# esologic/GANce

Hardware: AMD Instinct MI355X
Metric: synthesized frames/sec at 1024x1024 config-f (higher is better)
Workload: dtype f32 (bf16x3 split operands, 6 terms, fp32 accumulate)

## Files before the change

gance_amd/csrc/upfir_split.hip:

```cpp

#include <hip/hip_runtime.h>

#include <algorithm>
#include <cstdlib>
#include <cstring>
#include <type_traits>

#include "kernels.h"

#ifndef GANCE_UPFIRS_ABLATE
#define GANCE_UPFIRS_ABLATE 0
#endif

namespace gance {

namespace {

typedef float f32x4 __attribute__((ext_vector_type(4)));
typedef float f32x2 __attribute__((ext_vector_type(2)));
typedef unsigned u32x4 __attribute__((ext_vector_type(4)));
typedef __bf16 bf16x8 __attribute__((ext_vector_type(8)));
typedef __bf16 bf16x2 __attribute__((ext_vector_type(2)));
typedef __attribute__((address_space(3))) void* lds_ptr_t;

constexpr int kBM = 16;
constexpr int kKC = 32;
constexpr int kSW = 64;
constexpr int kTH = 8;
constexpr int kRows = kTH + 1;
constexpr int kPlanes = 12;
constexpr int kPlaneStride = 80;
constexpr int kSlotUnits = kPlanes * kPlaneStride;
constexpr int kRing = 3;
constexpr int kHaloCols = 4;
constexpr int kHaloUnits = kRows * kHaloCols * kPlanes;
constexpr int kHaloTasks = kRows * kHaloCols * 4;
#ifndef GANCE_UPFIRS_WEAVE
#define GANCE_UPFIRS_WEAVE 2
#endif
#ifndef GANCE_UPFIRS_MIN_SEG_ROWS
#define GANCE_UPFIRS_MIN_SEG_ROWS 16
#endif
#ifndef GANCE_UPFIRS_DEPTH
#define GANCE_UPFIRS_DEPTH 6
#endif
constexpr int kDepth = GANCE_UPFIRS_DEPTH;
constexpr int kCarryRows = 3;
constexpr int kPassCh = 4;
constexpr int kPassRows = 8;
constexpr int kTW = 2 * kSW + 4;
constexpr int kCG = kSW / 2;
constexpr int kRG = 64 / kCG;
constexpr int kFR = kPassRows / kRG;
constexpr int kWin = kFR + 3;
constexpr int kCarryFloats = kBM * kCarryRows * kTW;
constexpr int kStageFloats = kPassCh * kPassRows * kTW;
constexpr int kNzPieces = 2 * kPassRows * 2 * kSW / 256;
constexpr float kSqrt2f = 1.4142135623730951f;
static_assert((2 * kRows) % kDepth == 0 && kDepth + 2 < kRows && kRows % kRing == 0, "ring slots and staging registers rotate with the unrolled rows of a chunk pair");

constexpr size_t kRingBytes = (size_t)kRing * kSlotUnits * 16;
constexpr size_t kHaloBytes = (size_t)2 * kHaloUnits * 16;
constexpr int kWUnits = 27 * 64;
constexpr size_t kWBytes = (size_t)kWUnits * 16;
constexpr size_t lds_bytes(int cin) {
    return kRingBytes + kHaloBytes + kWBytes + sizeof(float) * ((size_t)kStageFloats + kNzPieces * 256 + kCarryFloats + cin + 3 * kBM);
}

__host__ __device__ constexpr int tap_cls(int t) { return t < 4 ? 0 : (t < 6 ? 1 : (t < 8 ? 2 : 3)); }
__host__ __device__ constexpr int tap_dy(int t) { return (t == 2 || t == 3 || t == 5) ? 1 : 0; }
__host__ __device__ constexpr int tap_dx(int t) { return (t == 1 || t == 3 || t == 7) ? 1 : 0; }

__device__ __forceinline__ void lds_barrier() {
    asm volatile("s_waitcnt lgkmcnt(0)" ::: "memory");
    __builtin_amdgcn_s_barrier();
    asm volatile("" ::: "memory");
}

__device__ __forceinline__ int fresh_lane() {
    int l;
    asm volatile("v_mbcnt_lo_u32_b32 %0, -1, 0\n\tv_mbcnt_hi_u32_b32 %0, -1, %0" : "=v"(l));
    return l;
}

__device__ __forceinline__ int ring_column(int P) {
    return ((P >> 2) & 3) | ((((P >> 4) ^ P) & 1) << 2) | (((P >> 1) & 1) << 3) | ((P & 1) << 4) | (P & 32);
}
constexpr int kEdgeColumn = 64;

__device__ __forceinline__ void split_pair(float a, float b, unsigned& p0, unsigned& p1, unsigned& p2) {
    auto pack = [](float lo, float hi) { return __builtin_bit_cast(unsigned, __builtin_convertvector(f32x2{lo, hi}, bf16x2)); };
    p0 = pack(a, b);
    const float ra = a - __builtin_bit_cast(float, p0 << 16), rb = b - __builtin_bit_cast(float, p0 & 0xffff0000u);
    p1 = pack(ra, rb);
    const float sa = ra - __builtin_bit_cast(float, p1 << 16), sb = rb - __builtin_bit_cast(float, p1 & 0xffff0000u);
    p2 = pack(sa, sb);
}

__device__ __forceinline__ void split_unit(const unsigned (&raw)[8], u32x4 (&part)[3]) {
    unsigned w[3][4];
    if (GANCE_UPFIRS_ABLATE & 1) {
#pragma unroll
        for (int q = 0; q < 3; ++q) part[q] = u32x4{raw[q], raw[q + 1], raw[q + 2], raw[q + 3]};
        return;
    }
#pragma unroll
    for (int e = 0; e < 4; ++e) split_pair(__builtin_bit_cast(float, raw[2 * e]), __builtin_bit_cast(float, raw[2 * e + 1]), w[0][e], w[1][e], w[2][e]);
#pragma unroll
    for (int q = 0; q < 3; ++q) part[q] = u32x4{w[q][0], w[q][1], w[q][2], w[q][3]};
}

}

template <bool kPre, bool kNoise>
__device__ __forceinline__ void upfirs_body(const UpFirArgs& p) {
    extern __shared__ __attribute__((aligned(16))) unsigned char smem_raw[];
    u32x4* const ring = reinterpret_cast<u32x4*>(smem_raw);
    u32x4* const halo = ring + kRing * kSlotUnits;
    u32x4* const w_lds = halo + 2 * kHaloUnits;
    float* const stage = reinterpret_cast<float*>(w_lds + kWUnits);
    float* const nz_lds = stage + kStageFloats;
    float* const carry = nz_lds + kNzPieces * 256;
    float* const s_lds = carry + kCarryFloats;
    float* const d_lds = s_lds + (kPre ? 0 : p.Cin);
    float* const b_lds = d_lds + kBM;
    float* const sn_lds = b_lds + kBM;

    const int tid = threadIdx.x;
    const int wave = __builtin_amdgcn_readfirstlane(tid >> 6);
    const int lane = tid & 63;
    const int n16 = lane & 15, kg = lane >> 4;

    int id;
    {
        const int v = blockIdx.x, nwg = p.total_blocks;
        const int q = nwg >> 3, r = nwg & 7, xcd = v & 7;
        id = (xcd < r ? xcd * (q + 1) : r * (q + 1) + (xcd - r) * q) + (v >> 3);
    }
    const int m_tile = id % p.m_tiles;
    id /= p.m_tiles;
    const int strip = id % p.strips;
    id /= p.strips;
    const int seg = id % p.segs;
    const int b = id / p.segs;
    const int m0 = m_tile * kBM;
    const int X0 = strip * kSW;
    const int H = p.H, W = p.W;
    const int Hp = H + 2, Wp = W + 8;
    const int HpWp4 = Hp * Wp * 4;
    const int chunks = p.Cin / kKC;
    const int steps = H / kTH;
    const int s_begin = seg * (p.rows_per_seg / kTH), s_end = s_begin + p.rows_per_seg / kTH;
    const int s_first = seg > 0 ? s_begin - 1 : s_begin;

    const __amdgpu_buffer_rsrc_t x_rsrc =
        __builtin_amdgcn_make_buffer_rsrc((void*)(p.x + (size_t)b * p.x_b_stride), 0, p.Cin * Hp * Wp * 4, 0x00020000);
    const __amdgpu_buffer_rsrc_t w_rsrc = __builtin_amdgcn_make_buffer_rsrc(
        (void*)(reinterpret_cast<const unsigned char*>(p.w) + (size_t)m_tile * chunks * 27 * 1024), 0, chunks * 27 * 1024, 0x00020000);

    const int st_pair = lane >> 4, st_g = lane & 15;
    u32x4* const ring_w = ring + wave * kPlaneStride + ring_column(4 * st_g + st_pair);
    const int m_pos = 16 * wave + n16;
    const u32x4* const ring_r0 = ring + kg * kPlaneStride + ring_column(m_pos);
    const u32x4* const ring_r1 = ring + kg * kPlaneStride + (m_pos > 0 ? ring_column(m_pos - 1) : kEdgeColumn);
    const bool edge_copy = wave == 3 && lane < kPlanes;
    const int e_unit = lane % kPlanes;
    u32x4* const ring_e = ring + (e_unit >> 2) * 4 * kPlaneStride + (e_unit & 3) * kPlaneStride + (edge_copy ? kEdgeColumn : 66 + wave);
    const u32x4* const halo_e = halo + e_unit;
    const u32x4* const halo_r = halo + ((n16 & 7) * kHaloCols + 2 * (n16 >> 3)) * kPlanes + kg;
    const u32x4* const halo_f = halo + ((kRows - 1) * kHaloCols + 2 * (n16 >> 3)) * kPlanes + kg;
    const int st_voff = (2 * st_pair * Hp * Wp + X0 + 4 + 4 * st_g) * 4;
    unsigned st[kDepth][8];
    auto stage_load = [&](unsigned(&dst)[8], int chunk, int brow, bool in_loop = false) {
        if ((GANCE_UPFIRS_ABLATE & 4) && in_loop) return;
        const int soff = ((chunk * kKC + wave * 8) * Hp + brow) * Wp * 4;
#pragma unroll
        for (int e = 0; e < 2; ++e) {
            const u32x4 q4 = __builtin_amdgcn_raw_buffer_load_b128(x_rsrc, st_voff, soff + e * HpWp4, 0);
#pragma unroll
            for (int c = 0; c < 4; ++c) dst[2 * c + e] = q4[c];
        }
    };
    auto scale_pair = [&](unsigned(&raw)[8], int chunk) {
        if constexpr (!kPre) {
            const f32x2 s2 = *reinterpret_cast<const f32x2*>(s_lds + chunk * kKC + 8 * wave + 2 * st_pair);
#pragma unroll
            for (int c = 0; c < 4; ++c) {
                raw[2 * c] = __builtin_bit_cast(unsigned, __builtin_bit_cast(float, raw[2 * c]) * s2[0]);
                raw[2 * c + 1] = __builtin_bit_cast(unsigned, __builtin_bit_cast(float, raw[2 * c + 1]) * s2[1]);
            }
        }
    };
    auto transpose_rows = [](u32x4& u) {
        auto a02 = __builtin_amdgcn_permlane32_swap(u[0], u[2], false, false);
        auto a13 = __builtin_amdgcn_permlane32_swap(u[1], u[3], false, false);
        auto b01 = __builtin_amdgcn_permlane16_swap(a02[0], a13[0], false, false);
        auto b23 = __builtin_amdgcn_permlane16_swap(a02[1], a13[1], false, false);
        u = u32x4{b01[0], b01[1], b23[0], b23[1]};
    };
    auto scale8 = [&](unsigned(&raw)[8], int chunk, int group) {
        if constexpr (!kPre) {
            const f32x4 s0 = *reinterpret_cast<const f32x4*>(s_lds + chunk * kKC + group * 8);
            const f32x4 s1 = *reinterpret_cast<const f32x4*>(s_lds + chunk * kKC + group * 8 + 4);
#pragma unroll
            for (int e = 0; e < 4; ++e) {
                raw[e] = __builtin_bit_cast(unsigned, __builtin_bit_cast(float, raw[e]) * s0[e]);
                raw[4 + e] = __builtin_bit_cast(unsigned, __builtin_bit_cast(float, raw[4 + e]) * s1[e]);
            }
        }
    };
    auto stage_store = [&](unsigned(&raw)[8], int slot, int chunk) {
        scale_pair(raw, chunk);
        u32x4 part[3];
        split_unit(raw, part);
#pragma unroll
        for (int q = 0; q < 3; ++q) transpose_rows(part[q]);
#pragma unroll
        for (int q = 0; q < 3; ++q)
            if (!(GANCE_UPFIRS_ABLATE & 16)) ring_w[slot * kSlotUnits + q * 4 * kPlaneStride] = part[q];
    };
    auto edge_store = [&](int slot, int hbuf, int hrow) { if (!(GANCE_UPFIRS_ABLATE & 64)) ring_e[slot * kSlotUnits] = halo_e[hbuf * kHaloUnits + (hrow * kHaloCols + 1) * kPlanes]; };
    const int h_task = tid < kHaloTasks ? tid : tid - kHaloTasks;
    const int h_col = h_task & 3, h_kg = (h_task >> 2) & 3, h_row = h_task >> 4;
    const int h_voff = ((h_kg * 8 * Hp + h_row) * Wp + X0 + 2 + (h_col & 1) + (h_col >> 1) * 65) * 4;
    u32x4* const halo_w = halo + (h_row * kHaloCols + h_col) * kPlanes + h_kg;
    unsigned hraw[8];
    auto halo_load = [&](int step, int chunk) {
        const int soff = (chunk * kKC * Hp + kTH * step) * Wp * 4;
#pragma unroll
        for (int e = 0; e < 8; ++e) hraw[e] = __builtin_amdgcn_raw_buffer_load_b32(x_rsrc, h_voff, soff + e * HpWp4, 0);
    };
    auto halo_store = [&](int chunk, int buf) {
        scale8(hraw, chunk, h_kg);
        u32x4 part[3];
        split_unit(hraw, part);
#pragma unroll
        for (int q = 0; q < 3; ++q) halo_w[buf * kHaloUnits + q * 4] = part[q];
    };

    u32x4 A[9][3];
    const int a_voff = lane * 16;
    auto weights_dma = [&](int chunk) {
#pragma unroll
        for (int k = 0; k < 7; ++k)
            if (k < 6 || wave < 3)
                __builtin_amdgcn_raw_ptr_buffer_load_lds(w_rsrc, (lds_ptr_t)(w_lds + (wave + 4 * k) * 64), 16, lane * 16, (chunk * 27 + wave + 4 * k) * 1024, 0, 0);
    };
    const u32x4* const w_r = w_lds + lane;
    auto read_a3 = [&](int t, u32x4(&dst)[3]) {
#pragma unroll
        for (int q = 0; q < 3; ++q) dst[q] = w_r[(t * 3 + q) * 64];
    };
    auto load_a3 = [&](int chunk, int t, u32x4(&dst)[3]) {
#pragma unroll
        for (int q = 0; q < 3; ++q) dst[q] = __builtin_amdgcn_raw_buffer_load_b128(w_rsrc, a_voff, (chunk * 27 + t * 3 + q) * 1024, 0);
    };

    u32x4 Bf[2][2][3];
    auto load_b = [&](int slot, u32x4(&dst)[2][3]) {
#pragma unroll
        for (int q = 0; q < 3; ++q) {
            dst[0][q] = ring_r0[slot * kSlotUnits + q * 4 * kPlaneStride];
            dst[1][q] = ring_r1[slot * kSlotUnits + q * 4 * kPlaneStride];
        }
    };

    stage_load(st[0], 0, kTH * s_first + 0);
    stage_load(st[1], 0, kTH * s_first + 1);
    load_a3(0, 0, A[0]);
    halo_load(s_first, 0);
    if constexpr (!kPre)
        for (int i = tid; i < p.Cin; i += 256) s_lds[i] = p.s[(size_t)b * p.s_stride + i];
    if (tid < kBM) {
        d_lds[tid] = p.d[(size_t)b * p.d_stride + m0 + tid];
        b_lds[tid] = p.bias[m0 + tid];
        sn_lds[tid] = p.s_next != nullptr ? p.s_next[(size_t)b * p.s_stride + m0 + tid] : 1.0f;
    }
    for (int i = tid; i < kCarryFloats; i += 256) carry[i] = 0.f;
#pragma unroll
    for (int t = 1; t < 9; ++t) load_a3(0, t, A[t]);
    if constexpr (!kPre) lds_barrier();
    stage_store(st[0], 0, 0);
    stage_store(st[1], 1, 0);
    halo_store(0, 0);
#pragma unroll
    for (int r = 2; r < 2 + kDepth; ++r) stage_load(st[r % kDepth], 0, kTH * s_first + r);
    lds_barrier();
    edge_store(0, 0, 0);
    edge_store(1, 0, 1);
    lds_barrier();
    load_b(0, Bf[0]);

    const int OW = 2 * W, OWp = OW + 8;
    const long long oplane = (long long)(2 * H + 2) * OWp;
    const __amdgpu_buffer_rsrc_t o_rsrc = __builtin_amdgcn_make_buffer_rsrc(
        (void*)(p.out + ((size_t)b * p.Cout + m0) * oplane - 2 * OWp), 0, 0x7fffffff, 0x00020000);
    const __amdgpu_buffer_rsrc_t nz_rsrc = __builtin_amdgcn_make_buffer_rsrc(
        (void*)(kNoise ? p.noise + (size_t)b * p.noise_b_stride : nullptr), 0, kNoise ? (2 * H) * (2 * W) * 4 : 0, 0x00020000);
    const float ns2 = p.noise_strength * kSqrt2f;

    constexpr int kTerms[6][2] = {{2, 0}, {0, 2}, {1, 1}, {1, 0}, {0, 1}, {0, 0}};
    constexpr int kTapTurn[9] = {0, 4, 6, 8, 2, 5, 1, 7, 3};

#pragma unroll 1
    for (int si = s_first; si < s_end; ++si) {
        const int y0 = kTH * si;
        const bool last_step = si + 1 == steps;
        const bool priming = si < s_begin;
        f32x4 acc[kTH][4];
#pragma unroll
        for (int r = 0; r < kTH; ++r)
#pragma unroll
            for (int c = 0; c < 4; ++c) acc[r][c] = f32x4{0.f, 0.f, 0.f, 0.f};
        f32x4 accf[2] = {f32x4{0.f, 0.f, 0.f, 0.f}, f32x4{0.f, 0.f, 0.f, 0.f}};
        f32x4 acch = f32x4{0.f, 0.f, 0.f, 0.f}, acchf = f32x4{0.f, 0.f, 0.f, 0.f};

        auto run_chunk = [&](auto parity, const int chunk) {
            constexpr int ab = decltype(parity)::value;
            const int n_chunk = chunk + 1 < chunks ? chunk + 1 : 0;
            const int n_step = chunk + 1 < chunks ? si : (last_step ? si : si + 1);
#pragma unroll
            for (int j = 0; j < kRows; ++j) {
                const int cur = (j + ab) & 1;
                if (j == 0) weights_dma(n_chunk);
                if (j == 0) halo_load(n_step, n_chunk);
                if (j == 4) halo_store(n_chunk, ab ^ 1);
                load_b((j + 1) % kRing, Bf[cur ^ 1]);
                edge_store((j + 2) % kRing, j + 2 < kRows ? ab : ab ^ 1, (j + 2) % kRows);
                stage_store(st[(kRows * ab + j + 2) % kDepth], (j + 2) % kRing, j + 2 < kRows ? chunk : n_chunk);
                stage_load(st[(kRows * ab + j + 2) % kDepth], j + 2 + kDepth < kRows ? chunk : n_chunk, kTH * (j + 2 + kDepth < kRows ? si : n_step) + (j + 2 + kDepth) % kRows, true);
                if (j + 1 < kRows) {
#pragma unroll
                    for (int term = 0; term < ((GANCE_UPFIRS_ABLATE & 8) ? 0 : 6); ++term)
#pragma unroll
                        for (int k = 0; k < 9; ++k) {
                            const int t = kTapTurn[k];
                            const int row = tap_dy(t) ? j : j - 1;
                            if (row < 0 || row >= kTH) continue;
                            acc[row][tap_cls(t)] = __builtin_amdgcn_mfma_f32_16x16x32_bf16(
                                __builtin_bit_cast(bf16x8, A[t][kTerms[term][1]]), __builtin_bit_cast(bf16x8, Bf[cur][tap_dx(t)][kTerms[term][0]]),
                                acc[row][tap_cls(t)], 0, 0, 0);
                        }
#pragma unroll
                    for (int i = 0; i < 54; ++i) {
                        if (i >= (j == 0 ? 18 : 54)) break;
                        __builtin_amdgcn_sched_group_barrier(0x008, 1, 0);
                        __builtin_amdgcn_sched_group_barrier(0x092, GANCE_UPFIRS_WEAVE, 0);
                    }
                } else {
                    constexpr int kOrder[9] = {2, 3, 5, 0, 1, 4, 6, 7, 8};
#pragma unroll
                    for (int i = 0; i < 9; ++i) {
                        const int t = kOrder[i];
                        if (!tap_dy(t)) {
#pragma unroll
                            for (int term = 0; term < 6; ++term)
                                acc[kTH - 1][tap_cls(t)] = __builtin_amdgcn_mfma_f32_16x16x32_bf16(
                                    __builtin_bit_cast(bf16x8, A[t][kTerms[term][1]]), __builtin_bit_cast(bf16x8, Bf[cur][tap_dx(t)][kTerms[term][0]]),
                                    acc[kTH - 1][tap_cls(t)], 0, 0, 0);
                        } else if (last_step) {
#pragma unroll
                            for (int term = 0; term < 6; ++term)
                                accf[tap_cls(t)] = __builtin_amdgcn_mfma_f32_16x16x32_bf16(
                                    __builtin_bit_cast(bf16x8, A[t][kTerms[term][1]]), __builtin_bit_cast(bf16x8, Bf[cur][tap_dx(t)][kTerms[term][0]]),
                                    accf[tap_cls(t)], 0, 0, 0);
                        }
                        if (wave == tap_cls(t) && !(GANCE_UPFIRS_ABLATE & 64)) {
                            u32x4 hf[3];
#pragma unroll
                            for (int q = 0; q < 3; ++q) hf[q] = halo_r[ab * kHaloUnits + ((1 - tap_dy(t)) * kHaloCols + 1 - tap_dx(t)) * kPlanes + q * 4];
#pragma unroll
                            for (int term = 0; term < 6; ++term)
                                acch = __builtin_amdgcn_mfma_f32_16x16x32_bf16(__builtin_bit_cast(bf16x8, A[t][kTerms[term][1]]),
                                                                               __builtin_bit_cast(bf16x8, hf[kTerms[term][0]]), acch, 0, 0, 0);
                            if (last_step && tap_dy(t)) {
#pragma unroll
                                for (int q = 0; q < 3; ++q) hf[q] = halo_f[ab * kHaloUnits + (1 - tap_dx(t)) * kPlanes + q * 4];
#pragma unroll
                                for (int term = 0; term < 6; ++term)
                                    acchf = __builtin_amdgcn_mfma_f32_16x16x32_bf16(__builtin_bit_cast(bf16x8, A[t][kTerms[term][1]]),
                                                                                    __builtin_bit_cast(bf16x8, hf[kTerms[term][0]]), acchf, 0, 0, 0);
                            }
                        }
                        read_a3(t, A[t]);
                    }
                }
                if (j == kRows - 2) asm volatile("s_waitcnt vmcnt(24)" ::: "memory");
                if (!(GANCE_UPFIRS_ABLATE & 32)) lds_barrier();
            }
        };
#pragma unroll 1
        for (int chunk = 0; chunk < chunks; chunk += 2) {
            run_chunk(std::integral_constant<int, 0>{}, chunk);
            run_chunk(std::integral_constant<int, 1>{}, chunk + 1);
        }

        const int elane = fresh_lane();
        const int en16 = elane & 15, eq4 = elane >> 4;
        const int dump_base = eq4 * (kPassRows * kTW) + 32 * wave + 2 * en16 + 1;
        const int hpy = wave >> 1, hpx = wave & 1;
        const int fc = wave;
        const int cg = elane % kCG;
        const int rg = elane / kCG;
        const int o_voff = (int)((fc * oplane + (long long)(kFR * rg) * OWp + 4 * cg) * 4);

        auto run_passes = [&](auto flush_tag) {
            constexpr bool kFlush = decltype(flush_tag)::value;
            const int ys = kFlush ? H : y0;
            if (kNoise) {
#pragma unroll
                for (int i = 0; i < kNzPieces / 4; ++i) {
                    const int f = (wave + 4 * i) * 256 + 4 * elane;
                    const int row = f / (2 * kSW), col = f % (2 * kSW);
                    __builtin_amdgcn_raw_ptr_buffer_load_lds(nz_rsrc, (lds_ptr_t)(nz_lds + (wave + 4 * i) * 256), 16,
                                                             ((2 * ys - 2 + row) * OW + 2 * X0 + col) * 4, 0, 0, 0);
                }
                asm volatile("s_waitcnt vmcnt(0)" ::: "memory");
            }
            constexpr int kRowPasses = kFlush ? 1 : 2;
#pragma unroll
            for (int rw = 0; rw < kRowPasses; ++rw) {
                const int oy0 = 2 * (ys + 4 * rw) - 2;
                const int r_lo = max(0, -oy0);
                const int r_hi = priming ? 0 : min(kPassRows, 2 * H - oy0);
#pragma unroll
                for (int g = 0; g < 4; ++g) {
                    if constexpr (kFlush) {
#pragma unroll
                        for (int c = 0; c < 4; ++c) stage[dump_base + (c >> 1) * kTW + (c & 1)] = c < 2 ? accf[c][g] : 0.f;
                        if (en16 == 0 || en16 == 8) {
                            const int side = en16 >> 3;
                            if (hpy == 0 && (side == 1 || hpx == 1)) stage[eq4 * (kPassRows * kTW) + (side ? 2 * kSW + 1 + hpx : 0)] = acchf[g];
                            if (hpy == 1 && (side == 1 || hpx == 1)) stage[eq4 * (kPassRows * kTW) + kTW + (side ? 2 * kSW + 1 + hpx : 0)] = 0.f;
                        }
                    } else {
#pragma unroll
                        for (int r4 = 0; r4 < 4; ++r4)
#pragma unroll
                            for (int c = 0; c < 4; ++c) stage[dump_base + (2 * r4 + (c >> 1)) * kTW + (c & 1)] = acc[4 * rw + r4][c][g];
                        const int row = en16 & 7, side = en16 >> 3;
                        if ((side == 1 || hpx == 1) && row / 4 == rw)
                            stage[eq4 * (kPassRows * kTW) + (2 * (row % 4) + hpy) * kTW + (side ? 2 * kSW + 1 + hpx : 0)] = acch[g];
                    }
                    lds_barrier();

                    const int ch = 4 * g + fc;
                    const float dsc = d_lds[ch] * kSqrt2f;
                    const float kh0 = 0.25f * dsc, kh1 = 0.75f * dsc;
                    const float bias2 = b_lds[ch] * kSqrt2f;
                    const float lr6 = 0.6f * sn_lds[ch], lr4 = 0.4f * sn_lds[ch];
                    const float* const win_lo = carry + ch * (kCarryRows * kTW) + (kFR * rg) * kTW + 4 * cg;
                    const float* const win_hi = stage + fc * (kPassRows * kTW) + (kFR * rg - kCarryRows) * kTW + 4 * cg;
                    f32x4 ta[kWin], tb[kWin];
#pragma unroll
                    for (int i = 0; i < kWin; ++i) {
                        const float* const rowp = (i < kCarryRows && kFR * rg + i < kCarryRows ? win_lo : win_hi) + i * kTW;
                        ta[i] = *reinterpret_cast<const f32x4*>(rowp);
                        tb[i] = *reinterpret_cast<const f32x4*>(rowp + 4);
                    }
                    {
                        const int o_soff = (int)((4 * g * oplane + (long long)(oy0 + 3) * OWp + 2 * X0 + 4) * 4);
#pragma unroll
                        for (int r = 0; r < kFR; ++r) {
                            const int rr = kFR * rg + r;
                            if (rr >= r_lo && rr < r_hi) {
                                f32x2 tv[4];
#pragma unroll
                                for (int c2 = 0; c2 < 4; ++c2) {
                                    auto pair = [&](int i) { return c2 < 2 ? f32x2{ta[i][2 * c2], ta[i][2 * c2 + 1]} : f32x2{tb[i][2 * c2 - 4], tb[i][2 * c2 - 3]}; };
                                    tv[c2] = 0.25f * pair(r) + 0.75f * pair(r + 1) + 0.75f * pair(r + 2) + 0.25f * pair(r + 3);
                                }
                                const float t[7] = {tv[0][0], tv[0][1], tv[1][0], tv[1][1], tv[2][0], tv[2][1], tv[3][0]};
                                f32x4 v;
#pragma unroll
                                for (int o = 0; o < 4; ++o) v[o] = fmaf(kh0, t[o + 3], fmaf(kh1, t[o + 2], fmaf(kh1, t[o + 1], fmaf(kh0, t[o], bias2))));
                                if (kNoise) v += ns2 * *reinterpret_cast<const f32x4*>(nz_lds + (kPassRows * rw + rr) * (2 * kSW) + 4 * cg);
#pragma unroll
                                for (int o = 0; o < 4; ++o) v[o] = fmaf(lr6, v[o], lr4 * __builtin_fabsf(v[o]));
                                if (!(GANCE_UPFIRS_ABLATE & 128)) __builtin_amdgcn_raw_buffer_store_b128(__builtin_bit_cast(u32x4, v), o_rsrc, o_voff, o_soff + r * OWp * 4, 0);
                                else asm volatile("" ::"v"(v));
                            }
                        }
                    }
                    lds_barrier();
                    if (!kFlush && rg == kRG - 1) {
                        float* const carry_w = carry + ch * (kCarryRows * kTW) + 4 * cg;
#pragma unroll
                        for (int i = 0; i < 3; ++i) {
                            *reinterpret_cast<f32x4*>(carry_w + i * kTW) = ta[kWin - 3 + i];
                            if (cg == kCG - 1) *reinterpret_cast<f32x4*>(carry_w + i * kTW + 4) = tb[kWin - 3 + i];
                        }
                    }
                }
            }
        };
        if (GANCE_UPFIRS_ABLATE & 2) {
            float sum = acch[0] + acchf[0] + accf[0][0] + accf[1][0];
#pragma unroll
            for (int r = 0; r < kTH; ++r)
#pragma unroll
                for (int c = 0; c < 4; ++c) sum += acc[r][c][0] + acc[r][c][3];
            if (sum == 12345.678f) p.out[tid] = sum;
            continue;
        }
        run_passes(std::false_type{});
        if (last_step) {
            lds_barrier();
            run_passes(std::true_type{});
        }
    }
}

bool upfirs_supported(int cin, int cout, int H, int W) {
    return H == W && W % kSW == 0 && H % kTH == 0 && cin % (2 * kKC) == 0 && cout % kBM == 0 && cin <= 512;
}

size_t upfirs_weight_floats(int cin, int cout) { return (size_t)(cout / kBM) * (cin / kKC) * 27 * 256; }

static unsigned short bf16_rne_host(float x) {
    unsigned u;
    std::memcpy(&u, &x, 4);
    u += 0x7fffu + ((u >> 16) & 1u);
    return (unsigned short)(u >> 16);
}
static float bf16_value_host(unsigned short h) {
    const unsigned u = (unsigned)h << 16;
    float f;
    std::memcpy(&f, &u, 4);
    return f;
}

void upfirs_arrange_weights(const float* w_in, int cin, int cout, const int* up_tap_weight, float* w_out) {
    unsigned short* const out = reinterpret_cast<unsigned short*>(w_out);
    const int m_tiles = cout / kBM, chunks = cin / kKC;
    for (int mt = 0; mt < m_tiles; ++mt)
        for (int ch = 0; ch < chunks; ++ch)
            for (int t = 0; t < 9; ++t)
                for (int k = 0; k < kKC; ++k)
                    for (int m = 0; m < kBM; ++m) {
                        const int channel = 4 * (m & 3) + (m >> 2);
                        const float v = w_in[((size_t)up_tap_weight[t] * cin + ch * kKC + k) * cout + mt * kBM + channel];
                        unsigned short part[3];
                        part[0] = bf16_rne_host(v);
                        const float r1 = v - bf16_value_host(part[0]);
                        part[1] = bf16_rne_host(r1);
                        part[2] = bf16_rne_host(r1 - bf16_value_host(part[1]));
                        for (int q = 0; q < 3; ++q)
                            out[((((((size_t)mt * chunks + ch) * 9 + t) * 3 + q) * 4 + k / 8) * 16 + m) * 8 + k % 8] = part[q];
                    }
}

void upfirs_plan(int B, int cout, int H, int W, int num_cus, UpFirArgs* a) {
    a->m_tiles = cout / kBM;
    a->strips = W / kSW;
    a->step_rows = kTH;
    static const bool segments = [] { const char* v = std::getenv("GANCE_TUNE_UPFIR_SPLIT_SEGS"); return !(v && std::atoi(v) == 0); }();
    int segs = 1;
    const int base = B * a->m_tiles * a->strips;
    long long best = (long long)((base + num_cus - 1) / num_cus) * H;
    for (int n = 2; segments && H / n >= GANCE_UPFIRS_MIN_SEG_ROWS && (H / n) % kTH == 0 && base * (n / 2) < num_cus; n *= 2) {
        const long long cost = (long long)((base * n + num_cus - 1) / num_cus) * (H / n + kTH);
        if (cost < best) best = cost, segs = n;
    }
    a->segs = segs;
    a->rows_per_seg = H / segs;
    a->total_blocks = base * segs;
    a->stagger_phases = 1;
    a->stagger_ticks = 0;
    a->debug_flags = 0;
}

__global__ __launch_bounds__(256, 1) void upfirs_fused_kernel(const UpFirArgs p) { upfirs_body<false, false>(p); }
__global__ __launch_bounds__(256, 1) void upfirs_fused_noise_kernel(const UpFirArgs p) { upfirs_body<false, true>(p); }
__global__ __launch_bounds__(256, 1) void upfirs_fused_pre_kernel(const UpFirArgs p) { upfirs_body<true, false>(p); }
__global__ __launch_bounds__(256, 1) void upfirs_fused_pre_noise_kernel(const UpFirArgs p) { upfirs_body<true, true>(p); }

hipError_t launch_upfir_split(const UpFirArgs& args, hipStream_t stream) {
    using Kernel = void (*)(const UpFirArgs);
    static const Kernel kernels[4] = {upfirs_fused_kernel, upfirs_fused_noise_kernel, upfirs_fused_pre_kernel, upfirs_fused_pre_noise_kernel};
    static PerDeviceInt ready;
    int unused = 0;
    const hipError_t e = ready.get(
        [&](int, int* value) {
            *value = 1;
            for (int i = 0; i < 4; ++i) {
                const hipError_t err =
                    hipFuncSetAttribute(reinterpret_cast<const void*>(kernels[i]), hipFuncAttributeMaxDynamicSharedMemorySize, (int)lds_bytes(i >= 2 ? 0 : 512));
                if (err != hipSuccess) return err;
            }
            return hipSuccess;
        },
        &unused);
    if (e != hipSuccess) return e;
    if (!upfirs_supported(args.Cin, args.Cout, args.H, args.W) || args.segs < 1 || args.rows_per_seg * args.segs != args.H || args.rows_per_seg % kTH != 0 ||
        args.total_blocks != args.B * args.m_tiles * args.strips * args.segs)
        return hipErrorInvalidValue;
    const int pre = args.input_prescaled ? 1 : 0, noise = args.noise != nullptr ? 1 : 0;
    hipLaunchKernelGGL(kernels[2 * pre + noise], dim3(args.total_blocks), dim3(256), lds_bytes(pre ? 0 : args.Cin), stream, args);
    return hipGetLastError();
}

}
```

Before: 1420.

## Compute upfirdn epilogue from accumulator registers via DPP instead of LDS staging passes

Replaces the staged epilogue, which dumped MFMA accumulators into an LDS stage buffer and ran two row-passes with barriers per channel group, with a register-resident filter. Neighbouring columns are exchanged with DPP row shifts, and only the tile-edge columns are published through a small LDS exchange buffer. Vertical carry rows are kept per lane, and priming or top-edge rows are suppressed by a zero-size buffer resource instead of branching. This cuts LDS traffic and the barriers in the epilogue. In exchange it relies on intricate lane and edge bookkeeping and adds register pressure, with accumulators forced into AGPRs.

```diff
diff --git a/gance_amd/csrc/upfir_split.hip b/gance_amd/csrc/upfir_split.hip
--- a/gance_amd/csrc/upfir_split.hip
+++ b/gance_amd/csrc/upfir_split.hip
@@ -46,16 +46,12 @@
 #endif
 constexpr int kDepth = GANCE_UPFIRS_DEPTH;
 constexpr int kCarryRows = 3;
-constexpr int kPassCh = 4;
-constexpr int kPassRows = 8;
-constexpr int kTW = 2 * kSW + 4;
-constexpr int kCG = kSW / 2;
-constexpr int kRG = 64 / kCG;
-constexpr int kFR = kPassRows / kRG;
-constexpr int kWin = kFR + 3;
-constexpr int kCarryFloats = kBM * kCarryRows * kTW;
-constexpr int kStageFloats = kPassCh * kPassRows * kTW;
-constexpr int kNzPieces = 2 * kPassRows * 2 * kSW / 256;
+constexpr int kXRows = 20;
+constexpr int kXSlots = 12;
+constexpr int kXFloats = kXSlots * kBM * kXRows;
+constexpr int kNzRows = 2 * kTH + 2;
+constexpr int kNzPieces = kNzRows * 2 * kSW / 256;
+constexpr int kCarryFloats = 4 * kCarryRows * 2 * 256;
 constexpr float kSqrt2f = 1.4142135623730951f;
 static_assert((2 * kRows) % kDepth == 0 && kDepth + 2 < kRows && kRows % kRing == 0, "ring slots and staging registers rotate with the unrolled rows of a chunk pair");
 
@@ -64,7 +60,7 @@
 constexpr int kWUnits = 27 * 64;
 constexpr size_t kWBytes = (size_t)kWUnits * 16;
 constexpr size_t lds_bytes(int cin) {
-    return kRingBytes + kHaloBytes + kWBytes + sizeof(float) * ((size_t)kStageFloats + kNzPieces * 256 + kCarryFloats + cin + 3 * kBM);
+    return kRingBytes + kHaloBytes + kWBytes + sizeof(float) * ((size_t)kXFloats + kNzPieces * 256 + kCarryFloats + cin + 3 * kBM);
 }
 
 __host__ __device__ constexpr int tap_cls(int t) { return t < 4 ? 0 : (t < 6 ? 1 : (t < 8 ? 2 : 3)); }
@@ -110,6 +106,12 @@
     for (int q = 0; q < 3; ++q) part[q] = u32x4{w[q][0], w[q][1], w[q][2], w[q][3]};
 }
 
+constexpr int kRowShr1 = 0x111, kRowShl1 = 0x101, kSwapPairs = 0xb1;
+template <int kCtrl>
+__device__ __forceinline__ float dpp(float old, float src) {
+    return __builtin_bit_cast(float, __builtin_amdgcn_update_dpp(__builtin_bit_cast(int, old), __builtin_bit_cast(int, src), kCtrl, 0xf, 0xf, false));
+}
+
 }
 
 template <bool kPre, bool kNoise>
@@ -118,8 +120,8 @@
     u32x4* const ring = reinterpret_cast<u32x4*>(smem_raw);
     u32x4* const halo = ring + kRing * kSlotUnits;
     u32x4* const w_lds = halo + 2 * kHaloUnits;
-    float* const stage = reinterpret_cast<float*>(w_lds + kWUnits);
-    float* const nz_lds = stage + kStageFloats;
+    float* const xbuf = reinterpret_cast<float*>(w_lds + kWUnits);
+    float* const nz_lds = xbuf + kXFloats;
     float* const carry = nz_lds + kNzPieces * 256;
     float* const s_lds = carry + kCarryFloats;
     float* const d_lds = s_lds + (kPre ? 0 : p.Cin);
@@ -295,6 +297,7 @@
     const long long oplane = (long long)(2 * H + 2) * OWp;
     const __amdgpu_buffer_rsrc_t o_rsrc = __builtin_amdgcn_make_buffer_rsrc(
         (void*)(p.out + ((size_t)b * p.Cout + m0) * oplane - 2 * OWp), 0, 0x7fffffff, 0x00020000);
+    const __amdgpu_buffer_rsrc_t o_rsrc_none = __builtin_amdgcn_make_buffer_rsrc(p.out, 0, 0, 0x00020000);
     const __amdgpu_buffer_rsrc_t nz_rsrc = __builtin_amdgcn_make_buffer_rsrc(
         (void*)(kNoise ? p.noise + (size_t)b * p.noise_b_stride : nullptr), 0, kNoise ? (2 * H) * (2 * W) * 4 : 0, 0x00020000);
     const float ns2 = p.noise_strength * kSqrt2f;
@@ -395,105 +398,6 @@
             run_chunk(std::integral_constant<int, 1>{}, chunk + 1);
         }
 
-        const int elane = fresh_lane();
-        const int en16 = elane & 15, eq4 = elane >> 4;
-        const int dump_base = eq4 * (kPassRows * kTW) + 32 * wave + 2 * en16 + 1;
-        const int hpy = wave >> 1, hpx = wave & 1;
-        const int fc = wave;
-        const int cg = elane % kCG;
-        const int rg = elane / kCG;
-        const int o_voff = (int)((fc * oplane + (long long)(kFR * rg) * OWp + 4 * cg) * 4);
-
-        auto run_passes = [&](auto flush_tag) {
-            constexpr bool kFlush = decltype(flush_tag)::value;
-            const int ys = kFlush ? H : y0;
-            if (kNoise) {
-#pragma unroll
-                for (int i = 0; i < kNzPieces / 4; ++i) {
-                    const int f = (wave + 4 * i) * 256 + 4 * elane;
-                    const int row = f / (2 * kSW), col = f % (2 * kSW);
-                    __builtin_amdgcn_raw_ptr_buffer_load_lds(nz_rsrc, (lds_ptr_t)(nz_lds + (wave + 4 * i) * 256), 16,
-                                                             ((2 * ys - 2 + row) * OW + 2 * X0 + col) * 4, 0, 0, 0);
-                }
-                asm volatile("s_waitcnt vmcnt(0)" ::: "memory");
-            }
-            constexpr int kRowPasses = kFlush ? 1 : 2;
-#pragma unroll
-            for (int rw = 0; rw < kRowPasses; ++rw) {
-                const int oy0 = 2 * (ys + 4 * rw) - 2;
-                const int r_lo = max(0, -oy0);
-                const int r_hi = priming ? 0 : min(kPassRows, 2 * H - oy0);
-#pragma unroll
-                for (int g = 0; g < 4; ++g) {
-                    if constexpr (kFlush) {
-#pragma unroll
-                        for (int c = 0; c < 4; ++c) stage[dump_base + (c >> 1) * kTW + (c & 1)] = c < 2 ? accf[c][g] : 0.f;
-                        if (en16 == 0 || en16 == 8) {
-                            const int side = en16 >> 3;
-                            if (hpy == 0 && (side == 1 || hpx == 1)) stage[eq4 * (kPassRows * kTW) + (side ? 2 * kSW + 1 + hpx : 0)] = acchf[g];
-                            if (hpy == 1 && (side == 1 || hpx == 1)) stage[eq4 * (kPassRows * kTW) + kTW + (side ? 2 * kSW + 1 + hpx : 0)] = 0.f;
-                        }
-                    } else {
-#pragma unroll
-                        for (int r4 = 0; r4 < 4; ++r4)
-#pragma unroll
-                            for (int c = 0; c < 4; ++c) stage[dump_base + (2 * r4 + (c >> 1)) * kTW + (c & 1)] = acc[4 * rw + r4][c][g];
-                        const int row = en16 & 7, side = en16 >> 3;
-                        if ((side == 1 || hpx == 1) && row / 4 == rw)
-                            stage[eq4 * (kPassRows * kTW) + (2 * (row % 4) + hpy) * kTW + (side ? 2 * kSW + 1 + hpx : 0)] = acch[g];
-                    }
-                    lds_barrier();
-
-                    const int ch = 4 * g + fc;
-                    const float dsc = d_lds[ch] * kSqrt2f;
-                    const float kh0 = 0.25f * dsc, kh1 = 0.75f * dsc;
-                    const float bias2 = b_lds[ch] * kSqrt2f;
-                    const float lr6 = 0.6f * sn_lds[ch], lr4 = 0.4f * sn_lds[ch];
-                    const float* const win_lo = carry + ch * (kCarryRows * kTW) + (kFR * rg) * kTW + 4 * cg;
-                    const float* const win_hi = stage + fc * (kPassRows * kTW) + (kFR * rg - kCarryRows) * kTW + 4 * cg;
-                    f32x4 ta[kWin], tb[kWin];
-#pragma unroll
-                    for (int i = 0; i < kWin; ++i) {
-                        const float* const rowp = (i < kCarryRows && kFR * rg + i < kCarryRows ? win_lo : win_hi) + i * kTW;
-                        ta[i] = *reinterpret_cast<const f32x4*>(rowp);
-                        tb[i] = *reinterpret_cast<const f32x4*>(rowp + 4);
-                    }
-                    {
-                        const int o_soff = (int)((4 * g * oplane + (long long)(oy0 + 3) * OWp + 2 * X0 + 4) * 4);
-#pragma unroll
-                        for (int r = 0; r < kFR; ++r) {
-                            const int rr = kFR * rg + r;
-                            if (rr >= r_lo && rr < r_hi) {
-                                f32x2 tv[4];
-#pragma unroll
-                                for (int c2 = 0; c2 < 4; ++c2) {
-                                    auto pair = [&](int i) { return c2 < 2 ? f32x2{ta[i][2 * c2], ta[i][2 * c2 + 1]} : f32x2{tb[i][2 * c2 - 4], tb[i][2 * c2 - 3]}; };
-                                    tv[c2] = 0.25f * pair(r) + 0.75f * pair(r + 1) + 0.75f * pair(r + 2) + 0.25f * pair(r + 3);
-                                }
-                                const float t[7] = {tv[0][0], tv[0][1], tv[1][0], tv[1][1], tv[2][0], tv[2][1], tv[3][0]};
-                                f32x4 v;
-#pragma unroll
-                                for (int o = 0; o < 4; ++o) v[o] = fmaf(kh0, t[o + 3], fmaf(kh1, t[o + 2], fmaf(kh1, t[o + 1], fmaf(kh0, t[o], bias2))));
-                                if (kNoise) v += ns2 * *reinterpret_cast<const f32x4*>(nz_lds + (kPassRows * rw + rr) * (2 * kSW) + 4 * cg);
-#pragma unroll
-                                for (int o = 0; o < 4; ++o) v[o] = fmaf(lr6, v[o], lr4 * __builtin_fabsf(v[o]));
-                                if (!(GANCE_UPFIRS_ABLATE & 128)) __builtin_amdgcn_raw_buffer_store_b128(__builtin_bit_cast(u32x4, v), o_rsrc, o_voff, o_soff + r * OWp * 4, 0);
-                                else asm volatile("" ::"v"(v));
-                            }
-                        }
-                    }
-                    lds_barrier();
-                    if (!kFlush && rg == kRG - 1) {
-                        float* const carry_w = carry + ch * (kCarryRows * kTW) + 4 * cg;
-#pragma unroll
-                        for (int i = 0; i < 3; ++i) {
-                            *reinterpret_cast<f32x4*>(carry_w + i * kTW) = ta[kWin - 3 + i];
-                            if (cg == kCG - 1) *reinterpret_cast<f32x4*>(carry_w + i * kTW + 4) = tb[kWin - 3 + i];
-                        }
-                    }
-                }
-            }
-        };
         if (GANCE_UPFIRS_ABLATE & 2) {
             float sum = acch[0] + acchf[0] + accf[0][0] + accf[1][0];
 #pragma unroll
@@ -503,10 +407,114 @@
             if (sum == 12345.678f) p.out[tid] = sum;
             continue;
         }
-        run_passes(std::false_type{});
-        if (last_step) {
-            lds_barrier();
-            run_passes(std::true_type{});
+        const int elane = fresh_lane();
+        const int en16 = elane & 15, eq4 = elane >> 4;
+        const int odd = en16 & 1;
+        const int hpy = wave >> 1, hpx = wave & 1;
+        auto xcol = [&](int slot, int ch) { return xbuf + (slot * kBM + ch) * kXRows; };
+        if (kNoise) {
+#pragma unroll
+            for (int i = 0; i < 3; ++i) {
+                const int piece = wave + 4 * i;
+                if (piece < 2 * kTH / 2 || (last_step && piece < kNzPieces)) {
+                    const int f = piece * 256 + 4 * elane;
+                    const int row = f / (2 * kSW), col = f % (2 * kSW);
+                    __builtin_amdgcn_raw_ptr_buffer_load_lds(nz_rsrc, (lds_ptr_t)(nz_lds + piece * 256), 16, ((2 * y0 - 2 + row) * OW + 2 * X0 + col) * 4, 0, 0, 0);
+                }
+            }
+        }
+        {
+            const bool pub_l = en16 == 15 && wave < 3, pub_r = en16 == 0 && wave > 0;
+            if (pub_l || pub_r) {
+                float* const x1 = xcol(pub_l ? wave + 1 : 5 + 2 * (wave - 1), eq4);
+                float* const x0 = xcol(4 + 2 * (wave - 1), eq4);
+#pragma unroll
+                for (int g = 0; g < 4; ++g) {
+#pragma unroll
+                    for (int a = 0; a < 4; ++a) {
+                        *reinterpret_cast<f32x4*>(x1 + 4 * g * kXRows + 4 * a) = f32x4{acc[2 * a][1][g], acc[2 * a][3][g], acc[2 * a + 1][1][g], acc[2 * a + 1][3][g]};
+                        if (pub_r) *reinterpret_cast<f32x4*>(x0 + 4 * g * kXRows + 4 * a) = f32x4{acc[2 * a][0][g], acc[2 * a][2][g], acc[2 * a + 1][0][g], acc[2 * a + 1][2][g]};
+                    }
+                    if (last_step) {
+                        x1[4 * g * kXRows + 2 * kTH] = accf[1][g];
+                        if (pub_r) x0[4 * g * kXRows + 2 * kTH] = accf[0][g];
+                    }
+                }
+            }
+            const int hrow = en16 & 7, side = en16 >> 3;
+            if (side == 1 || hpx == 1) {
+                float* const xh = xcol(side ? 10 + hpx : 0, eq4) + 2 * hrow + hpy;
+#pragma unroll
+                for (int g = 0; g < 4; ++g) xh[4 * g * kXRows] = acch[g];
+                if (last_step && hpy == 0 && hrow == 0)
+#pragma unroll
+                    for (int g = 0; g < 4; ++g) xh[4 * g * kXRows + 2 * kTH] = acchf[g];
+            }
+        }
+        if (kNoise) asm volatile("s_waitcnt vmcnt(0)" ::: "memory");
+        lds_barrier();
+#pragma unroll
+        for (int r = 0; r < kTH; ++r)
+#pragma unroll
+            for (int c = 0; c < 4; ++c) asm volatile("" : "+a"(acc[r][c]));
+
+        const __amdgpu_buffer_rsrc_t o_rsrc_step = priming ? o_rsrc_none : o_rsrc;
+        const __amdgpu_buffer_rsrc_t o_rsrc_first = y0 == 0 ? o_rsrc_none : o_rsrc_step;
+        f32x2* const carry_l = reinterpret_cast<f32x2*>(carry) + tid;
+        const int o_voff = (int)((eq4 * oplane + (long long)odd * OWp + 2 * X0 + 32 * wave + 4 * (en16 >> 1) + 4) * 4);
+        const float* const x_old = xcol(en16 == 0 ? wave : 4 + 2 * wave, eq4);
+        const float* const nz_r = nz_lds + 2 * (16 * wave + en16);
+#pragma unroll
+        for (int g = 0; g < 4; ++g) {
+            const int ch = 4 * g + eq4;
+            const float dsc = d_lds[ch] * kSqrt2f;
+            const f32x2 kh0 = 0.25f * dsc, kh1 = 0.75f * dsc;
+            const f32x2 bias2 = b_lds[ch] * kSqrt2f;
+            const float lr6 = 0.6f * sn_lds[ch], lr4 = 0.4f * sn_lds[ch];
+            f32x2 w0 = carry_l[(3 * g + 0) * 256], w1 = carry_l[(3 * g + 1) * 256], w2 = carry_l[(3 * g + 2) * 256];
+            f32x2 v_even;
+            auto t_row = [&](const int i) {
+                f32x2 h = 0.f;
+                if (i <= 2 * kTH) {
+                    const float old1 = x_old[4 * g * kXRows + i], old2 = x_old[(kBM + 4 * g) * kXRows + i];
+                    const float c0 = i < 2 * kTH ? acc[i / 2][2 * (i % 2)][g] : accf[0][g];
+                    const float c1 = i < 2 * kTH ? acc[i / 2][2 * (i % 2) + 1][g] : accf[1][g];
+                    const float l = dpp<kRowShr1>(old1, c1), r0 = dpp<kRowShl1>(old1, c0), r1 = dpp<kRowShl1>(old2, c1);
+                    h = __builtin_elementwise_fma(kh0, f32x2{r0, r1}, __builtin_elementwise_fma(kh1, f32x2{c1, r0}, __builtin_elementwise_fma(kh1, f32x2{c0, c1}, kh0 * f32x2{l, c0})));
+                    if (i >= 2 * kTH - kCarryRows && i < 2 * kTH) carry_l[(3 * g + i - (2 * kTH - kCarryRows)) * 256] = h;
+                }
+                {
+                    f32x2 v = __builtin_elementwise_fma(f32x2(0.25f), h, __builtin_elementwise_fma(f32x2(0.75f), w2, __builtin_elementwise_fma(f32x2(0.75f), w1, __builtin_elementwise_fma(f32x2(0.25f), w0, bias2))));
+                    if (kNoise) {
+                        const f32x2 nz = *reinterpret_cast<const f32x2*>(nz_r + i * (2 * kSW));
+                        v[0] = fmaf(ns2, nz[0], v[0]);
+                        v[1] = fmaf(ns2, nz[1], v[1]);
+                    }
+                    if (i % 2 == 0) {
+                        v_even = v;
+                    } else {
+                        const f32x2 send = odd ? v_even : v;
+                        const f32x2 recv = f32x2{dpp<kSwapPairs>(0.f, send[0]), dpp<kSwapPairs>(0.f, send[1])};
+                        f32x4 o = odd ? f32x4{recv[0], recv[1], v[0], v[1]} : f32x4{v_even[0], v_even[1], recv[0], recv[1]};
+#pragma unroll
+                        for (int e = 0; e < 4; ++e) o[e] = fmaf(lr6, o[e], lr4 * __builtin_fabsf(o[e]));
+                        const int o_soff = (int)((4 * g * oplane + (long long)(2 * y0 - 2 + i - 1 + 3) * OWp) * 4);
+                        if (!(GANCE_UPFIRS_ABLATE & 128)) __builtin_amdgcn_raw_buffer_store_b128(__builtin_bit_cast(u32x4, o), i == 1 ? o_rsrc_first : o_rsrc_step, o_voff, o_soff, 0);
+                        else asm volatile("" ::"v"(o));
+                    }
+                }
+                w0 = w1;
+                w1 = w2;
+                w2 = h;
+                if (i % 2 == 1) __builtin_amdgcn_sched_barrier(0);
+            };
+#pragma unroll
+            for (int i = 0; i < 2 * kTH; ++i) t_row(i);
+            if (last_step) {
+                t_row(2 * kTH);
+                t_row(2 * kTH + 1);
+            }
+            __builtin_amdgcn_sched_barrier(0);
         }
     }
 }
```

New measurement: 1433 (median of 6 runs). Within noise of the previous version (+1.0%).
